# alibaba/unified-audio

Measured on AMD Instinct MI355X. Metric: audio-seconds/sec H-Codec encode+decode @16kHz b=32, higher is better.
Workload: dtype f32

## Files before the change

unified_audio_amd/csrc/conv_gemm.hip:

```cpp
#include <algorithm>
#include <cstdlib>
#include <type_traits>

#include "common.h"
#include "split_planes.h"

#ifndef QA_LOAD_AT
#define QA_LOAD_AT 0
#endif

#ifdef QA_TIMING
__device__ unsigned long long g_qa_timing[10];
extern "C" int qa_debug_timing(unsigned long long* out, int reset) {
    if (out && hipMemcpyFromSymbol(out, HIP_SYMBOL(g_qa_timing), sizeof(g_qa_timing)) != hipSuccess) return -1;
    if (reset) {
        unsigned long long z[10] = {0};
        if (hipMemcpyToSymbol(HIP_SYMBOL(g_qa_timing), z, sizeof(z)) != hipSuccess) return -1;
    }
    return 0;
}
#endif

namespace qa {

__host__ __device__ constexpr int conv_gemm_lds_bytes(int BM, int BN, int BK, bool split) {
    return (split ? 2 * (BM + BN) * 3 * BK * 2 : 2 * (BM + BN) * (BK + 4) * 4) + BM * 8 * 4;
}
__host__ __device__ constexpr int conv_gemm_min_wg(int BM, int BN, int BK, bool split) {
    const int regs = BM == 256 ? (BK == 16 ? 2 : 1) : (BM == 64 && (BK == 16 || BN == 64) ? 4 : (BK == 16 ? 3 : 2));
    const int lds = 160 * 1024 / conv_gemm_lds_bytes(BM, BN, BK, split);
    return regs < lds ? regs : (lds < 1 ? 1 : lds);
}

template <int N, int I = 0, class F>
__device__ __forceinline__ void static_for(F&& f) {
    if constexpr (I < N) {
        f(std::integral_constant<int, I>{});
        static_for<N, I + 1>(f);
    }
}

constexpr int TAP_WIN = 8;

__device__ __forceinline__ float snake_f(float x, float a) {
    const float s = sinf(a * x);
    return x + s * s / (a + 1e-9f);
}
__device__ __forceinline__ f32x4 snake4(f32x4 v, const float* alpha, int n) {
    const f32x4 a = *reinterpret_cast<const f32x4*>(alpha + n);
    const f32x4 r = {snake_f(v.x, a.x), snake_f(v.y, a.y), snake_f(v.z, a.z), snake_f(v.w, a.w)};
    return r;
}

__device__ __forceinline__ f32x4 epilogue4(f32x4 v, const ConvParams& p, long long m, int n, f32x4 bias, f32x4 gamma) {
    v += bias;
    if (p.gate) {
        const f32x4 g = *reinterpret_cast<const f32x4*>(p.gate + m * p.ldg + n);
        v.x *= silu_f(g.x); v.y *= silu_f(g.y); v.z *= silu_f(g.z); v.w *= silu_f(g.w);
    }
    if (p.act == ACT_SNAKE) {
        v = snake4(v, p.alpha, n);
    } else if (p.act != ACT_NONE) {
        v.x = apply_act(v.x, p.act); v.y = apply_act(v.y, p.act); v.z = apply_act(v.z, p.act); v.w = apply_act(v.w, p.act);
    }
    if (p.gamma) v *= gamma;
    if (p.res) v += *reinterpret_cast<const f32x4*>(p.res + m * p.ldr + n);
    if (p.post_act == ACT_SNAKE) {
        v = snake4(v, p.alpha, n);
    } else if (p.post_act != ACT_NONE) {
        v.x = apply_act(v.x, p.post_act); v.y = apply_act(v.y, p.post_act); v.z = apply_act(v.z, p.post_act);
        v.w = apply_act(v.w, p.post_act);
    }
    if (p.y2) *reinterpret_cast<f32x4*>(p.y2 + m * p.ldy2 + n) = snake4(v, p.alpha2, n);
    if (p.rope && n < p.rope_n) {
        const int t = p.rope_pos0 + (int)(m % p.rope_T), i = (n % p.rope_hd) >> 1;
        const f32x4 cs = *reinterpret_cast<const f32x4*>(p.rope + ((long long)t * (p.rope_hd >> 1) + i) * 2);
        const f32x4 r = {v.x * cs.x - v.y * cs.y, v.y * cs.x + v.x * cs.y, v.z * cs.z - v.w * cs.w, v.w * cs.z + v.z * cs.w};
        v = r;
    }
    return v;
}

template <int BM, int BN, int WM, int WN, bool PRO_ELU, int BK = 32, bool LINEAR = false, int NPL = 0, bool PRE = false>
__global__ __launch_bounds__(256, conv_gemm_min_wg(BM, BN, BK, NPL > 0)) void conv_gemm_kernel(const ConvParams p_in) {
    constexpr bool SPLIT = NPL > 0;
    constexpr int NP = SPLIT ? NPL : 3;
    static_assert(NPL >= 0 && NPL <= 3, "0 = fp32 chain, else the number of bf16 planes");
    static_assert(SPLIT || !PRE, "a pre-split weight image feeds the bf16-plane instances only");
    ConvParams p = p_in;
    constexpr int CK = SPLIT ? 32 : BK;
    constexpr bool ONE_BUF = SPLIT && BK == 16;
    constexpr int LDS = BK + 4;
    constexpr int RPP = 256 / (CK / 4);
    constexpr int WTM = BM / WM, WTN = BN / WN;
    constexpr int TM = WTM / 32, TN = WTN / 32;
    constexpr int A_IT = BM / RPP, B_IT = BN / RPP;
    static_assert(WM * WN == 4, "4 waves per workgroup");
    static_assert(TM >= 1 && TN >= 1, "wave tile must hold at least one 32x32 MFMA tile");

    constexpr int SMEM_FLOATS = SPLIT ? (ONE_BUF ? 1 : 2) * (BM + BN) * 3 * CK / 2 : 2 * (BM + BN) * LDS;
    __shared__ __attribute__((aligned(16))) float smem[SMEM_FLOATS];
    __shared__ int s_tap[BM * TAP_WIN];
    float* sA = smem;
    float* sB = smem + 2 * BM * LDS;
    constexpr int PLANE_A = BM * CK * 2, PLANE_B = BN * CK * 2;
    constexpr int BUF_BYTES = 3 * (PLANE_A + PLANE_B);
    char* const sbytes = reinterpret_cast<char*>(smem);
    auto swz = [](int row, int slot) { return slot ^ ((0 - (row >> 2)) & 3); };

    const int tid = threadIdx.x, lane = tid & 63, wave = tid >> 6;
    const int wm = wave / WN, wn = wave % WN;
    const int tiles_n = (p.N + BN - 1) / BN;
    int tile = blockIdx.x;
    if (p.xcd_swizzle) {
        const int nwg = gridDim.x, q = nwg >> 3, r = nwg & 7;
        const int xcd = tile & 7, local = tile >> 3;
        tile = (xcd < r ? xcd * (q + 1) : r * (q + 1) + (xcd - r) * q) + local;
    }
    int tm_i = tile / tiles_n, tn_i = tile % tiles_n;
    if (p.panel > 0 && tiles_n > p.panel) {
        const int tiles_m = (p.M + BM - 1) / BM;
        const int per_panel = tiles_m * p.panel;
        const int panel = tile / per_panel, r = tile - panel * per_panel;
        const int pw = min(p.panel, tiles_n - panel * p.panel);
        tm_i = r / pw;
        tn_i = panel * p.panel + (r - tm_i * pw);
    }
    const int m0 = tm_i * BM;
    const int n0 = tn_i * BN;

    const int ld_row = tid / (CK / 4);
    const int ld_c4 = (tid % (CK / 4)) * 4;
    const bool ld_hi = SPLIT && ld_c4 >= 16, bp_hi = (tid & 2) != 0;
    const bool k_tail = SPLIT && (p.K & 16) != 0;

    const bool reflect = p.pad_mode == PAD_REFLECT;
    const int ldx_i = (int)p.ldx;
    const int t_virtual = p.T_in * (p.in_rep > 1 ? p.in_rep : 1);
    const int dil = p.dilation > 1 ? p.dilation : 1;
    auto build_taps = [&](int jbase) {
        for (int e = tid; e < BM * TAP_WIN; e += 256) {
            const int row = e / TAP_WIN, j = jbase + (e % TAP_WIN);
            const int m = min(m0 + row, p.M - 1);
            const int t = m % p.T_out;
            int len = t_virtual, lp = p.Lp;
            if (p.lens) {
                len = min(p.lens[m / p.T_out] * p.len_mul, t_virtual);
                lp = len <= p.max_pad ? p.max_pad + 1 : len;
            }
            int r = t * p.stride - p.pad_left + j * dil;
            const int rr = r < 0 ? -r : (r >= lp ? 2 * (lp - 1) - r : r);
            r = reflect ? rr : r;
            const bool ok = r >= 0 && r < len && j < p.ksize;
            const unsigned ru = ok ? (unsigned)r : 0u;
            const unsigned src = __umulhi(ru, p.rep_magic) + ru * p.rep_one;
            s_tap[e] = ok ? (int)(src * (unsigned)ldx_i) : -1;
        }
    };
    if (!LINEAR) build_taps(0);
    int jbase = 0;

    const float* a_ptr[A_IT];
    int a_tab[A_IT];
#pragma unroll
    for (int i = 0; i < A_IT; ++i) {
        const int m = min(m0 + ld_row + RPP * i, p.M - 1);
        a_ptr[i] = LINEAR ? p.x + (long long)m * p.ldx + ld_c4 : p.x + (long long)(m / p.T_out) * p.T_in * p.ldx + ld_c4;
        a_tab[i] = (ld_row + RPP * i) * TAP_WIN;
    }
    const float* b_ptr[B_IT];
    if constexpr (!PRE) {
#pragma unroll
        for (int i = 0; i < B_IT; ++i) {
            const int n = min(n0 + ld_row + RPP * i, p.N - 1);
            b_ptr[i] = p.w + (long long)n * p.K + ld_c4;
        }
    }
    constexpr int BP_BLOCK = 16 * NP;
    constexpr int BP_UNITS = BN * CK / 128 * BP_BLOCK, BP_IT = PRE ? BP_UNITS / 256 : 1;
    static_assert(!PRE || (BN == 128 && BP_UNITS % 256 == 0), "the image path exists for the 128-column tiles: every thread moves BP_IT whole units");
    const char* bp_ptr[BP_IT];
    int bp_lds[BP_IT];
    if constexpr (PRE) {
#pragma unroll
        for (int i = 0; i < BP_IT; ++i) {
            const int u = tid + 256 * i, v = u % BP_BLOCK;
            const int pl = v >> 4, slot = v % (CK / 8);
            const int row = u / BP_BLOCK * (128 / CK) + (v & 15) / (CK / 8);
            const int n = min(n0 + row, p.N - 1);
            bp_ptr[i] = static_cast<const char*>(p.wp) + plane_byte_offset((long long)n * p.K + slot * 8, pl);
            bp_lds[i] = 3 * PLANE_A + pl * PLANE_B + row * CK * 2 + swz(row, slot) * 16;
        }
    }
    const int nk = (p.K + CK - 1) / CK;

    f32x16 acc[TM][TN];
#pragma unroll
    for (int i = 0; i < TM; ++i)
#pragma unroll
        for (int j = 0; j < TN; ++j)
#pragma unroll
            for (int r = 0; r < 16; ++r) acc[i][j][r] = 0.f;
    constexpr int TM16 = WTM / 16, TN16 = WTN / 16;
    f32x4 acc4[SPLIT ? TM16 : 1][SPLIT ? TN16 : 1];
    if constexpr (SPLIT) {
#pragma unroll
        for (int i = 0; i < TM16; ++i)
#pragma unroll
            for (int j = 0; j < TN16; ++j) acc4[i][j] = f32x4{0.f, 0.f, 0.f, 0.f};
    }

    f32x4 a_reg[A_IT], b_reg[B_IT];
    u32x4 bp_reg[BP_IT];
    float a_keep[A_IT];

#define QA_LOAD_GLOBAL(KC)                                                                                     \
    {                                                                                                          \
        const int k0_ = (KC) * CK;                                                                             \
        const bool tl_ = k_tail && (KC) == nk - 1;             \
        const int kt_ = k0_ - (tl_ && ld_hi ? 16 : 0);          \
        if (LINEAR) {                                                                                          \
            _Pragma("unroll") for (int i = 0; i < A_IT; ++i) a_reg[i] = *reinterpret_cast<const f32x4*>(a_ptr[i] + kt_); \
        } else {                                                                                               \
            const int j0_ = k0_ / p.C_in;                                                                      \
            const int c0_ = k0_ - j0_ * p.C_in;                                                                \
            int j1_ = j0_, c1_ = c0_;                                                                          \
            if (SPLIT && (p.C_in & 16)) {        \
                const int kh_ = tl_ ? k0_ : k0_ + 16;                                                          \
                j1_ = kh_ / p.C_in;                                                                            \
                c1_ = kh_ - j1_ * p.C_in - 16;                                                                 \
            }                                                                                                  \
            if (j1_ >= jbase + TAP_WIN) {                         \
                jbase = j0_;                                                                                   \
                build_taps(jbase);                                                                             \
                __syncthreads();                                                                               \
            }                                                                                                  \
            const int j_ = ld_hi ? j1_ : j0_, c_ = ld_hi ? c1_ : c0_;                                          \
            _Pragma("unroll") for (int i = 0; i < A_IT; ++i) {                                                 \
                const int off_ = s_tap[a_tab[i] + (j_ - jbase)];                                               \
                a_keep[i] = off_ >= 0 ? 1.f : 0.f;                                                             \
                a_reg[i] = *reinterpret_cast<const f32x4*>(a_ptr[i] + (max(off_, 0) + c_));                    \
            }                                                                                                  \
        }                                                                                                      \
        if constexpr (PRE) {                                                                                   \
            const long long bo_ = (long long)(KC) * (CK * 6) - (tl_ && bp_hi ? 2 * PLANE_GROUP_BYTES : 0);     \
            _Pragma("unroll") for (int i = 0; i < BP_IT; ++i)                                                  \
                bp_reg[i] = *reinterpret_cast<const u32x4*>(bp_ptr[i] + bo_);                                  \
        } else {                                                                                               \
            _Pragma("unroll") for (int i = 0; i < B_IT; ++i) b_reg[i] = *reinterpret_cast<const f32x4*>(b_ptr[i] + kt_); \
        }                                                                                                      \
    }
#define QA_STORE_LDS(BUF, KC)                                                                                  \
    { if constexpr (SPLIT) {                                                                                   \
        char* a_ = sbytes + (BUF) * BUF_BYTES;                                                                 \
        const int sl_ = ld_c4 >> 3, in_ = (ld_c4 & 7) * 2;                                                     \
        if (k_tail && (KC) == nk - 1) {        \
            const f32x4 z4_ = {0.f, 0.f, 0.f, 0.f};                                                            \
            const u32x4 zu_ = {0u, 0u, 0u, 0u};                                                                \
            _Pragma("unroll") for (int i = 0; i < A_IT; ++i) a_reg[i] = ld_hi ? z4_ : a_reg[i];                \
            if constexpr (PRE) {                                                                               \
                _Pragma("unroll") for (int i = 0; i < BP_IT; ++i) bp_reg[i] = bp_hi ? zu_ : bp_reg[i];         \
            } else {                                                                                           \
                _Pragma("unroll") for (int i = 0; i < B_IT; ++i) b_reg[i] = ld_hi ? z4_ : b_reg[i];            \
            }                                                                                                  \
        }                                                                                                      \
        _Pragma("unroll") for (int i = 0; i < A_IT; ++i) {                                                     \
            f32x4 v = LINEAR ? a_reg[i] : a_reg[i] * a_keep[i];                                                \
            if (PRO_ELU) {                                                                                     \
                v.x = elu_f(v.x); v.y = elu_f(v.y); v.z = elu_f(v.z); v.w = elu_f(v.w);                        \
            }                                                                                                  \
            u32x2 h_, m_, l_;                                                                                  \
            split4_planes<NP>(v, h_, m_, l_);                                                                  \
            const int r_ = ld_row + RPP * i, o_ = r_ * CK * 2 + swz(r_, sl_) * 16 + in_;                       \
            *reinterpret_cast<u32x2*>(a_ + o_) = h_;                                                           \
            if constexpr (NP >= 2) *reinterpret_cast<u32x2*>(a_ + PLANE_A + o_) = m_;                          \
            if constexpr (NP == 3) *reinterpret_cast<u32x2*>(a_ + 2 * PLANE_A + o_) = l_;                      \
        }                                                                                                      \
        if constexpr (PRE) {                                                                                   \
            _Pragma("unroll") for (int i = 0; i < BP_IT; ++i)                                                  \
                *reinterpret_cast<u32x4*>(a_ + bp_lds[i]) = bp_reg[i];                                         \
        } else {                                                                                               \
        char* b_ = a_ + 3 * PLANE_A;                                                                           \
        _Pragma("unroll") for (int i = 0; i < B_IT; ++i) {                                                     \
            u32x2 h_, m_, l_;                                                                                  \
            split4_planes<NP>(b_reg[i], h_, m_, l_);                                                           \
            const int r_ = ld_row + RPP * i, o_ = r_ * CK * 2 + swz(r_, sl_) * 16 + in_;                       \
            *reinterpret_cast<u32x2*>(b_ + o_) = h_;                                                           \
            if constexpr (NP >= 2) *reinterpret_cast<u32x2*>(b_ + PLANE_B + o_) = m_;                          \
            if constexpr (NP == 3) *reinterpret_cast<u32x2*>(b_ + 2 * PLANE_B + o_) = l_;                      \
        } }                                                                                                    \
    } else {                                                                                                   \
        float* a_ = sA + (BUF) * BM * LDS;                                                                     \
        float* b_ = sB + (BUF) * BN * LDS;                                                                     \
        _Pragma("unroll") for (int i = 0; i < A_IT; ++i) {                                                     \
            f32x4 v = LINEAR ? a_reg[i] : a_reg[i] * a_keep[i];                                                \
            if (PRO_ELU) {                                                                                     \
                v.x = elu_f(v.x); v.y = elu_f(v.y); v.z = elu_f(v.z); v.w = elu_f(v.w);                        \
            }                                                                                                  \
            *reinterpret_cast<f32x4*>(a_ + (ld_row + RPP * i) * LDS + ld_c4) = v;                              \
        }                                                                                                      \
        _Pragma("unroll") for (int i = 0; i < B_IT; ++i)                                                       \
            *reinterpret_cast<f32x4*>(b_ + (ld_row + RPP * i) * LDS + ld_c4) = b_reg[i];                       \
    } }

    __syncthreads();
    QA_LOAD_GLOBAL(0)
    QA_STORE_LDS(0, 0)
    __syncthreads();

    const int frag_row = lane & 31;
    const int frag_k = (lane >> 5) * 4;
#ifdef QA_TIMING
    const long long tbegin = __builtin_readcyclecounter();
    const unsigned long long rbegin = __builtin_amdgcn_s_memrealtime();
#endif
    constexpr int NKK = BK / 8;
    if constexpr (SPLIT) {
        constexpr int RB = BM == 256 ? 4 : 1;
        constexpr int STORE_J = TN16 > 1 ? 1 : 0;
        const int fr = lane & 15, sl = lane >> 4;
        int a_off[TM16], b_off[TN16];
#pragma unroll
        for (int i = 0; i < TM16; ++i) {
            const int r = wm * WTM + i * 16 + fr;
            a_off[i] = r * CK * 2 + swz(r, sl) * 16;
        }
#pragma unroll
        for (int j = 0; j < TN16; ++j) {
            const int r = wn * WTN + j * 16 + fr;
            b_off[j] = 3 * PLANE_A + r * CK * 2 + swz(r, sl) * 16;
        }
        for (int kc = 0; kc < nk; ++kc) {
            const int cur = ONE_BUF ? 0 : kc & 1;
            const int nxt = min(kc + 1, nk - 1);
            const char* base = sbytes + cur * BUF_BYTES;
            QA_LOAD_GLOBAL(nxt)
            static_for<RB>([&](auto rb_c) {
                constexpr int i0 = decltype(rb_c)::value * (TM16 / RB);
                bf16x8 af[NP][TM16 / RB];
#pragma unroll
                for (int pl = 0; pl < NP; ++pl)
#pragma unroll
                    for (int i = 0; i < TM16 / RB; ++i) af[pl][i] = *reinterpret_cast<const bf16x8*>(base + pl * PLANE_A + a_off[i0 + i]);
#pragma unroll
                for (int j = 0; j < TN16; ++j) {
                    bf16x8 bf[NP];
#pragma unroll
                    for (int pl = 0; pl < NP; ++pl) bf[pl] = *reinterpret_cast<const bf16x8*>(base + pl * PLANE_B + b_off[j]);
                    if (!ONE_BUF && i0 + TM16 / RB == TM16 && j == STORE_J) QA_STORE_LDS(cur ^ 1, nxt)
                    static_for<6>([&](auto q_c) {
                        constexpr int q = decltype(q_c)::value;
                        if constexpr (pair_kept(q, NP)) {
#pragma unroll
                            for (int i = 0; i < TM16 / RB; ++i)
                                acc4[i0 + i][j] = __builtin_amdgcn_mfma_f32_16x16x32_bf16(bf[PAIR_B[q]], af[PAIR_A[q]][i], acc4[i0 + i][j], 0, 0, 0);
                        }
                    });
                }
            });
            __builtin_amdgcn_sched_barrier(0);
            if constexpr (ONE_BUF) {
                if (kc + 1 < nk) {
                    __syncthreads();
                    QA_STORE_LDS(0, nxt)
                    __syncthreads();
                }
            } else {
                __syncthreads();
            }
        }
    } else
    for (int kc = 0; kc < nk; ++kc) {
        const int cur = kc & 1;
        const int nxt = min(kc + 1, nk - 1);
        const float* a = sA + cur * BM * LDS + (wm * WTM + frag_row) * LDS + frag_k;
        const float* b = sB + cur * BN * LDS + (wn * WTN + frag_row) * LDS + frag_k;
        f32x4 af[2][TM], bf[2][TN];
#pragma unroll
        for (int i = 0; i < TM; ++i) af[0][i] = *reinterpret_cast<const f32x4*>(a + i * 32 * LDS);
#pragma unroll
        for (int j = 0; j < TN; ++j) bf[0][j] = *reinterpret_cast<const f32x4*>(b + j * 32 * LDS);
#pragma unroll
        for (int kk = 0; kk < NKK; ++kk) {
            const int cb = kk & 1, nb = cb ^ 1;
            if (kk < NKK - 1) {
#pragma unroll
                for (int i = 0; i < TM; ++i) af[nb][i] = *reinterpret_cast<const f32x4*>(a + i * 32 * LDS + (kk + 1) * 8);
#pragma unroll
                for (int j = 0; j < TN; ++j) bf[nb][j] = *reinterpret_cast<const f32x4*>(b + j * 32 * LDS + (kk + 1) * 8);
            }
            if (kk == QA_LOAD_AT) QA_LOAD_GLOBAL(nxt)
            if (kk == NKK - 1) QA_STORE_LDS(cur ^ 1, nxt)
#pragma unroll
            for (int i = 0; i < TM; ++i)
#pragma unroll
                for (int j = 0; j < TN; ++j) {
                    acc[i][j] = __builtin_amdgcn_mfma_f32_32x32x2f32(bf[cb][j].x, af[cb][i].x, acc[i][j], 0, 0, 0);
                    acc[i][j] = __builtin_amdgcn_mfma_f32_32x32x2f32(bf[cb][j].y, af[cb][i].y, acc[i][j], 0, 0, 0);
                    acc[i][j] = __builtin_amdgcn_mfma_f32_32x32x2f32(bf[cb][j].z, af[cb][i].z, acc[i][j], 0, 0, 0);
                    acc[i][j] = __builtin_amdgcn_mfma_f32_32x32x2f32(bf[cb][j].w, af[cb][i].w, acc[i][j], 0, 0, 0);
                }
            __builtin_amdgcn_sched_barrier(0);
        }
        __syncthreads();
    }
#ifdef QA_TIMING
    const long long tloop = __builtin_readcyclecounter();
#endif
#undef QA_LOAD_GLOBAL
#undef QA_STORE_LDS

    constexpr int EP_LD = BN + 4;
    constexpr int EP_ROWS = WM * 32;
    constexpr int EP_C4 = BN / 4;
    static_assert(EP_ROWS * EP_LD <= 2 * (BM + BN) * LDS, "epilogue staging must fit in the operand buffers");
    static_assert(256 % EP_C4 == 0, "a thread keeps its column group across iterations");
    static_assert(EP_C4 % 8 == 0, "arg-min epilogue: the 8 lanes of a 32-column group are consecutive lanes of one wave");
    float* stage = smem;
    const int row_l = lane & 31, col_h = 4 * (lane >> 5);
    const int ep_c4 = tid % EP_C4, ep_r0 = tid / EP_C4;
    const int ep_n = n0 + 4 * ep_c4;
    const f32x4 zero4 = {0.f, 0.f, 0.f, 0.f}, one4 = {1.f, 1.f, 1.f, 1.f};
    f32x4 bias4 = zero4, gamma4 = one4;
    if (p.vec_epi && ep_n < p.N) {
        if (p.bias) bias4 = *reinterpret_cast<const f32x4*>(p.bias + ep_n);
        if (p.gamma) gamma4 = *reinterpret_cast<const f32x4*>(p.gamma + ep_n);
    }
    static_for<TM>([&](auto i_c) {
        constexpr int i = decltype(i_c)::value;
        __syncthreads();
        if constexpr (SPLIT) {
#pragma unroll
            for (int h = 0; h < 2; ++h)
#pragma unroll
                for (int j = 0; j < TN16; ++j)
                    *reinterpret_cast<f32x4*>(stage + (wm * 32 + h * 16 + (lane & 15)) * EP_LD + wn * WTN + j * 16 + 4 * (lane >> 4)) = acc4[2 * i + h][j];
        } else {
#pragma unroll
        for (int j = 0; j < TN; ++j)
#pragma unroll
            for (int g = 0; g < 4; ++g) {
                const f32x4 v = {acc[i][j][4 * g], acc[i][j][4 * g + 1], acc[i][j][4 * g + 2], acc[i][j][4 * g + 3]};
                *reinterpret_cast<f32x4*>(stage + (wm * 32 + row_l) * EP_LD + wn * WTN + j * 32 + 8 * g + col_h) = v;
            }
        }
        __syncthreads();
#pragma unroll 1
        for (int r = ep_r0; r < EP_ROWS; r += 256 / EP_C4) {
            const long long m = m0 + (r >> 5) * WTM + i * 32 + (r & 31);
            if (p.am_dist) {
                float best = INFINITY;
                int bi = 0x7fffffff;
                if (m < p.M && ep_n < p.N) {
                    const f32x4 sv = *reinterpret_cast<const f32x4*>(stage + r * EP_LD + 4 * ep_c4);
                    const f32x4 e4 = *reinterpret_cast<const f32x4*>(p.am_e2 + ep_n);
                    const float xx = p.am_x2[m];
#pragma unroll
                    for (int e = 0; e < 4; ++e) {
                        const float dist = (xx - 2.f * sv[e]) + e4[e];
                        if (dist < best) {
                            best = dist;
                            bi = ep_n + e;
                        }
                    }
                }
#pragma unroll
                for (int o = 1; o < 8; o <<= 1) {
                    const float d2 = __shfl_xor(best, o, 64);
                    const int i2 = __shfl_xor(bi, o, 64);
                    if (d2 < best || (d2 == best && i2 < bi)) {
                        best = d2;
                        bi = i2;
                    }
                }
                if ((ep_c4 & 7) == 0 && m < p.M && ep_n < p.N) {
                    p.am_dist[m * p.am_ld + (ep_n >> 5)] = best;
                    p.am_idx[m * p.am_ld + (ep_n >> 5)] = bi;
                }
                continue;
            }
            if (m >= p.M || ep_n >= p.N) continue;
            f32x4 v = *reinterpret_cast<const f32x4*>(stage + r * EP_LD + 4 * ep_c4);
            if (p.vec_epi) {
                v = epilogue4(v, p, m, ep_n, bias4, gamma4);
                *reinterpret_cast<f32x4*>(p.y + m * p.ldy + ep_n) = v;
            } else {
                for (int e = 0; e < 4 && ep_n + e < p.N; ++e) {
                    const int n = ep_n + e;
                    float u = v[e] + (p.bias ? p.bias[n] : 0.f);
                    if (p.gate) u = silu_f(p.gate[m * p.ldg + n]) * u;
                    u = apply_act(u, p.act);
                    if (p.gamma) u *= p.gamma[n];
                    if (p.res) u += p.res[m * p.ldr + n];
                    u = apply_act(u, p.post_act);
                    p.y[m * p.ldy + n] = u;
                }
            }
        }
    });
#ifdef QA_TIMING
    if (lane == 0) {
        const long long tend = __builtin_readcyclecounter();
        atomicAdd(&g_qa_timing[4], (unsigned long long)(tend - tloop));
        atomicAdd(&g_qa_timing[5], (unsigned long long)(tend - tbegin));
        atomicAdd(&g_qa_timing[6], 1ULL);
        atomicAdd(&g_qa_timing[7], (unsigned long long)nk);
        atomicAdd(&g_qa_timing[8], __builtin_amdgcn_s_memrealtime() - rbegin);
    }
#endif
}

static bool is_linear(const ConvParams& p) {
    return knob(K_GEMM_LINEAR) != 0 && p.ksize == 1 && p.stride == 1 && p.pad_left == 0 && p.in_rep <= 1 && p.T_in == p.T_out && p.dilation <= 1;
}

constexpr int prof_cfg(int bm, int bn) {
    return bm == 256 ? PROF_CFG_256x128 : bm == 64 ? (bn == 64 ? PROF_CFG_64x64 : PROF_CFG_64x128) : bn == 32 ? PROF_CFG_128x32 : bn == 64 ? PROF_CFG_128x64 : PROF_CFG_128x128;
}

static int gemm_planes(const ConvParams& p) {
    const long long math = knob(K_GEMM_MATH);
    return math == 0 || p.math_fp32 ? 0 : math == 2 ? 2 : math == 3 ? 1 : 3;
}

template <int BM, int BN, int WM, int WN, bool ELU, int BK, bool LIN>
static void launch_instance(const ConvParams& p, long long tiles, hipStream_t stream) {
    constexpr bool IMAGE = BN == 128;
    const bool image = IMAGE && p.wp;
    void (*kernel)(const ConvParams) = nullptr;
    switch (gemm_planes(p)) {
        case 0: kernel = conv_gemm_kernel<BM, BN, WM, WN, ELU, BK, LIN, 0, false>; break;
        case 1: kernel = image ? conv_gemm_kernel<BM, BN, WM, WN, ELU, BK, LIN, 1, IMAGE> : conv_gemm_kernel<BM, BN, WM, WN, ELU, BK, LIN, 1, false>; break;
        case 2: kernel = image ? conv_gemm_kernel<BM, BN, WM, WN, ELU, BK, LIN, 2, IMAGE> : conv_gemm_kernel<BM, BN, WM, WN, ELU, BK, LIN, 2, false>; break;
        default: kernel = image ? conv_gemm_kernel<BM, BN, WM, WN, ELU, BK, LIN, 3, IMAGE> : conv_gemm_kernel<BM, BN, WM, WN, ELU, BK, LIN, 3, false>; break;
    }
    hipLaunchKernelGGL(kernel, dim3((unsigned)tiles), dim3(256), 0, stream, p);
}

static thread_local int t_gemm_lanes = 1;
GemmLanes::GemmLanes(int n) : prev(t_gemm_lanes) { t_gemm_lanes = n > 1 ? n : 1; }
GemmLanes::~GemmLanes() { t_gemm_lanes = prev; }
static bool takes_bk16(int bm, int bn, long long tiles, int K, int C_in, bool elu) {
    return bm == 256 ||
           (bn >= 64 && !elu && ((K <= knob(K_GEMM_BK16) && tiles * t_gemm_lanes >= knob(K_GEMM_BK16_MIN_TILES)) || C_in % 32 != 0));
}

template <int BM, int BN, int WM, int WN>
static int launch_cfg(const ConvParams& p, hipStream_t stream) {
    QA_REQUIRE(p.prologue == ACT_NONE || p.prologue == ACT_ELU, "conv_gemm: prologue %d unsupported", p.prologue);
    const long long tiles = ceil_div(p.M, BM) * ceil_div(p.N, BN);
    const bool linear = is_linear(p), elu = p.prologue == ACT_ELU;
    const bool bk16 = takes_bk16(BM, BN, tiles, p.K, p.C_in, elu);
    const int bk = bk16 || gemm_planes(p) > 0 ? 16 : 32;
    const bool table = BM != 256 && (!linear || elu);
    QA_REQUIRE(p.K % bk == 0 && (!table || p.C_in % bk == 0),
               "conv_gemm: the %dx%d tile's K chunk needs K=%d / C_in=%d to be multiples of %d", BM, BN, p.K, p.C_in, bk);
    const bool prof = profile_enabled();
    if (prof) {
        const double n = p.algo_n ? p.algo_n : p.N, k = p.algo_k ? p.algo_k : p.K;
        const double out_elems = p.am_dist ? 2.0 * (double)p.M * p.am_ld + p.M + n
                                            : (double)p.M * n * (1.0 + (p.res ? 1.0 : 0.0) + (p.gate ? 1.0 : 0.0));
        const double elems = (double)p.B * p.T_in * p.C_in + n * k + out_elems;
        profile_record_begin(prof_cfg(BM, BN), 2.0 * (double)p.M * n * k, 4.0 * elems, stream, &p);
    }
    if constexpr (BM == 256) QA_REQUIRE(linear && !elu, "conv_gemm: the 256 x 128 tile exists for LINEAR layers only");
    constexpr int BK16 = BN >= 64 ? 16 : 32;
    if (bk16 && linear) launch_instance<BM, BN, WM, WN, false, BK16, true>(p, tiles, stream);
    else if constexpr (BM != 256) {
        if (bk16) launch_instance<BM, BN, WM, WN, false, BK16, false>(p, tiles, stream);
        else if (elu) launch_instance<BM, BN, WM, WN, true, 32, false>(p, tiles, stream);
        else if (linear) launch_instance<BM, BN, WM, WN, false, 32, true>(p, tiles, stream);
        else launch_instance<BM, BN, WM, WN, false, 32, false>(p, tiles, stream);
    }
    if (prof) profile_record_end(stream);
    QA_LAUNCH_CHECK();
    return QA_OK;
}

struct TileQuery {
    long long M, N, K;
    int C_in;
    bool lin, elu, split;
    bool image;
    int share;
};
static int workgroups_per_cu(int cfg, bool bk16, bool split) {
    switch (cfg) {
        case PROF_CFG_128x128: return bk16 ? 3 : split ? 1 : 2;
        case PROF_CFG_64x128: return bk16 ? 4 : 2;
        case PROF_CFG_128x64: return bk16 ? 4 : 2;
        case PROF_CFG_64x64: return bk16 ? 5 : split ? 3 : 4;
        case PROF_CFG_256x128: return 2;
        default: return split ? 2 : 3;
    }
}
static double tile_cost(const TileQuery& t, int cfg, int bm, int bn, double eff) {
    constexpr double kTile = 128.0 * 128.0, kRamp = 0.22, kLaunch = 0.27 * 512.0;
    const long long tiles = ceil_div(t.M, bm) * ceil_div(t.N, bn);
    const long long w = workgroups_per_cu(cfg, takes_bk16(bm, bn, tiles, (int)t.K, t.C_in, t.elu), t.split);
    const long long n = tiles * (t.share > 1 ? t.share : 1), cap = 256 * w;
    const long long rounds = ceil_div(n, cap), m = n - (rounds - 1) * cap;
    double last = 0.5 * ((double)ceil_div(m, 256) + (double)m / 256.0);
    if (last < 1.0) last = 1.0;
    return kTile * kLaunch + (double)t.K * ((double)bm * bn / eff * ((double)(w * (rounds - 1)) + last) + kRamp * kTile * (double)rounds);
}
static double tile_cost_r4(const TileQuery& t, int bm, int bn, double eff) {
    const long long tiles = ceil_div(t.M, bm) * ceil_div(t.N, bn);
    return (double)ceil_div(tiles, 256) * bm * bn / eff * (tiles <= 256 ? 1.25 : 1.0);
}
static int choose_tile(const TileQuery& t) {
    int cfg = (int)knob(K_GEMM_CFG);
    if (cfg < 0) {
        if (t.N <= 32) cfg = PROF_CFG_128x32;
        else if (t.N <= 64) cfg = PROF_CFG_128x64;
        else {
            struct Cand { int cfg, bm, bn; double eff6, eff32; };
            static const Cand cands[] = {{PROF_CFG_128x128, 128, 128, 1.0, 1.0}, {PROF_CFG_64x128, 64, 128, 0.85, 0.914},
                                         {PROF_CFG_128x64, 128, 64, 0.80, 0.913}, {PROF_CFG_64x64, 64, 64, 0.69, 0.871}};
            double best = 0.0;
            cfg = PROF_CFG_128x128;
            const long long eff256 = knob(K_GEMM_256);
            const bool r4 = t.split && !t.image;
            if (eff256 > 0 && t.lin && t.M >= 8000 && t.N >= 1024) {
                best = r4 ? tile_cost_r4(t, 256, 128, eff256 / 1000.0) : tile_cost(t, PROF_CFG_256x128, 256, 128, eff256 / 1000.0);
                cfg = PROF_CFG_256x128;
            }
            for (const Cand& c : cands) {
                const double cost = r4 ? tile_cost_r4(t, c.bm, c.bn, c.eff32) : tile_cost(t, c.cfg, c.bm, c.bn, t.split ? c.eff6 : c.eff32);
                if (best == 0.0 || cost < best * 0.995) {
                    best = cost;
                    cfg = c.cfg;
                }
            }
        }
    }
    if (cfg == PROF_CFG_128x32 && t.C_in % 32 != 0) return PROF_CFG_128x64;
    if ((cfg == PROF_CFG_256x128 && !t.lin) || cfg >= PROF_NCFG) return PROF_CFG_128x128;
    return cfg;
}
static int choose_tile(const ConvParams& p) {
    const bool elu = p.prologue == ACT_ELU;
    return choose_tile(TileQuery{p.M, p.N, p.K, p.C_in, is_linear(p) && !elu, elu, knob(K_GEMM_MATH) != 0 && !p.math_fp32, p.wp != nullptr, 1});
}

int launch_conv_gemm(const ConvParams& p, hipStream_t stream) {
    QA_REQUIRE(p.K % 16 == 0 && p.C_in % 16 == 0, "conv_gemm: K=%d / C_in=%d must be multiples of 16", p.K, p.C_in);
    QA_REQUIRE(p.C_in % 32 == 0 || gemm_planes(p) > 0 || (p.N > 32 && p.prologue != ACT_ELU),
               "conv_gemm: C_in=%d is not a multiple of 32 (the fp32 chain supports that only for N > 32 without the ELU prologue)", p.C_in);
    QA_REQUIRE((p.ldx % 4) == 0, "conv_gemm: ldx=%lld must be a multiple of 4 floats", p.ldx);
    QA_REQUIRE((long long)p.T_in * p.ldx < (1LL << 31), "conv_gemm: one batch item spans %lld floats (limit 2^31)",
               (long long)p.T_in * p.ldx);
    QA_REQUIRE(((uintptr_t)p.x % 16) == 0 && ((uintptr_t)p.w % 16) == 0, "conv_gemm: x / w must be 16-byte aligned");
    if (p.M <= 0 || p.N <= 0) return QA_OK;
    QA_REQUIRE(ceil_div(p.M, 64) * ceil_div(p.N, 32) < (1LL << 31), "conv_gemm: grid too large");
    auto al16 = [](const void* ptr) { return ((uintptr_t)ptr % 16) == 0; };
    const bool vec_epi = p.N % 4 == 0 && p.ldy % 4 == 0 && al16(p.y) && (!p.bias || al16(p.bias)) && (!p.gamma || al16(p.gamma)) &&
                         (!p.res || (p.ldr % 4 == 0 && al16(p.res))) && (!p.gate || (p.ldg % 4 == 0 && al16(p.gate)));
    QA_REQUIRE(p.in_rep <= 1 || p.pad_mode == PAD_ZERO, "conv_gemm: in_rep needs zero padding");
    const bool snake = p.act == ACT_SNAKE || p.post_act == ACT_SNAKE;
    QA_REQUIRE((!snake && !p.y2) || (vec_epi && (!snake || (p.alpha && al16(p.alpha))) &&
                                     (!p.y2 || (p.alpha2 && al16(p.alpha2) && al16(p.y2) && p.ldy2 % 4 == 0))),
               "conv_gemm: Snake activation / second output need the float4 epilogue and 16-byte aligned alpha vectors");
    QA_REQUIRE(p.dilation <= 1 || (p.pad_mode == PAD_ZERO && p.in_rep <= 1), "conv_gemm: dilation needs zero padding");
    QA_REQUIRE(!p.lens || (p.len_mul >= 1 && p.max_pad >= 0), "conv_gemm: per-clip lengths need len_mul >= 1");
    QA_REQUIRE(!p.am_dist || (vec_epi && p.am_idx && p.am_x2 && p.am_e2 && al16(p.am_e2) && p.am_ld >= (p.N + 31) / 32 && !p.y2),
               "conv_gemm: the arg-min epilogue needs N %% 4 == 0, x2 / e2 / dist / idx and am_ld >= ceil(N / 32)");
    QA_REQUIRE(!p.rope || (vec_epi && p.rope_hd % 4 == 0 && p.rope_n % 4 == 0 && p.rope_T > 0 && al16(p.rope)),
               "conv_gemm: fused RoPE needs the float4 epilogue (N, strides, pointers multiples of 4 / 16 B)");
    ConvParams q = p;
    q.xcd_swizzle = (int)knob(K_GEMM_XCD);
    q.panel = (int)knob(K_GEMM_PANEL);
    q.wp = knob(K_GEMM_PRESPLIT) != 0 ? weight_planes_find(p.w, (long long)p.N * p.K) : nullptr;
    q.vec_epi = vec_epi;
    q.rep_one = p.in_rep > 1 ? 0u : 1u;
    q.rep_magic = p.in_rep > 1 ? (unsigned)(((1ULL << 32) + p.in_rep - 1) / p.in_rep) : 0u;

    switch (choose_tile(q)) {
        case PROF_CFG_128x32: return launch_cfg<128, 32, 4, 1>(q, stream);
        case PROF_CFG_128x64: return launch_cfg<128, 64, 2, 2>(q, stream);
        case PROF_CFG_64x128: return launch_cfg<64, 128, 1, 4>(q, stream);
        case PROF_CFG_64x64: return launch_cfg<64, 64, 2, 2>(q, stream);
        case PROF_CFG_256x128: return launch_cfg<256, 128, 2, 2>(q, stream);
        default: return launch_cfg<128, 128, 2, 2>(q, stream);
    }
}

int conv_params_from_args(const qa_conv_args& a, ConvParams* out) {
    ConvParams p{};
    QA_REQUIRE(a.x && a.w && a.y, "conv1d_cl: x, w, y must be non-null");
    QA_REQUIRE(a.B > 0 && a.T_in > 0 && a.C_in > 0 && a.N > 0 && a.T_out >= 0, "conv1d_cl: bad shape");
    QA_REQUIRE(a.ksize >= 1 && a.stride >= 1 && a.pad_left >= 0 && a.pad_right >= 0, "conv1d_cl: bad geometry");
    QA_REQUIRE(a.B * a.T_out < (1LL << 31) && a.ksize * a.C_in < (1LL << 31), "conv1d_cl: shape too large");
    p.x = a.x; p.w = a.w; p.bias = a.bias; p.gamma = a.gamma; p.res = a.residual; p.gate = a.gate; p.y = a.y;
    p.ldx = a.ldx ? a.ldx : a.C_in;
    p.ldy = a.ldy ? a.ldy : a.N;
    p.ldr = a.ldr ? a.ldr : a.N;
    p.ldg = a.ldg ? a.ldg : a.N;
    p.B = (int)a.B; p.T_in = (int)a.T_in; p.C_in = (int)a.C_in; p.T_out = (int)a.T_out; p.N = (int)a.N;
    p.K = (int)(a.ksize * a.C_in);
    p.M = (int)(a.B * a.T_out);
    p.ksize = a.ksize; p.stride = a.stride; p.pad_left = a.pad_left; p.pad_mode = a.pad_mode;
    const int max_pad = a.pad_left > a.pad_right ? a.pad_left : a.pad_right;
    p.Lp = (p.T_in <= max_pad) ? max_pad + 1 : p.T_in;
    p.in_rep = a.in_rep > 1 ? a.in_rep : 1;
    QA_REQUIRE(a.T_out == 0 || (a.T_out - 1) * (int64_t)a.stride + a.ksize <= a.pad_left + a.T_in * (int64_t)p.in_rep + a.pad_right,
               "conv1d_cl: T_out=%lld windows do not fit pad_left=%d + T_in=%lld + pad_right=%d", (long long)a.T_out,
               a.pad_left, (long long)a.T_in, a.pad_right);
    p.prologue = a.prologue; p.act = a.act; p.post_act = a.post_act;
    *out = p;
    return QA_OK;
}

}

extern "C" int qa_debug_conv_gemm_tile(long long M, long long N, long long K, int ksize, int linear, int math_fp32, int share) {
    if (M <= 0 || N <= 0 || K <= 0 || ksize < 1 || K % ksize != 0 || M >= (1LL << 31) || N >= (1LL << 31) || K >= (1LL << 31)) {
        qa::set_error("qa_debug_conv_gemm_tile: bad argument");
        return -1;
    }
    const bool lin = linear != 0 && ksize == 1 && qa::knob(qa::K_GEMM_LINEAR) != 0;
    return qa::choose_tile(qa::TileQuery{M, N, K, (int)(K / ksize), lin, false, qa::knob(qa::K_GEMM_MATH) != 0 && !math_fp32, true, share});
}
```

Baseline: 3496.

## Fold clip offsets into tap table and pack padding mask into one register

The tap table now stores the full offset relative to the tile's first clip, so the conv A-loader keeps a single base pointer instead of A_IT per-row pointers and row-table indices. The per-row float keep factors become bits in one mask register, set with alignbit and applied as a select instead of a multiply. Separately, ELU-prologue 128x128 split layers may now take the BK16 instance. A host check keeps tile offsets within 32 bits, and a debug entry point is added. This is meant to cut VGPR pressure and address arithmetic in the hot load loop. The risk is that the new BK16 ELU instances behave differently or fail the offset limit on large inputs.

After: 3556, median of 6. 1.7% higher.

```diff
diff --git a/unified_audio_amd/csrc/conv_gemm.hip b/unified_audio_amd/csrc/conv_gemm.hip
--- a/unified_audio_amd/csrc/conv_gemm.hip
+++ b/unified_audio_amd/csrc/conv_gemm.hip
@@ -3,6 +3,7 @@
 #include <type_traits>
 
 #include "common.h"
+#include "conv_offsets.h"
 #include "split_planes.h"
 
 #ifndef QA_LOAD_AT
@@ -138,14 +139,16 @@
     const int ldx_i = (int)p.ldx;
     const int t_virtual = p.T_in * (p.in_rep > 1 ? p.in_rep : 1);
     const int dil = p.dilation > 1 ? p.dilation : 1;
+    const int clip0 = m0 / p.T_out;
+    const unsigned clip_stride = (unsigned)p.T_in * (unsigned)ldx_i;
     auto build_taps = [&](int jbase) {
         for (int e = tid; e < BM * TAP_WIN; e += 256) {
             const int row = e / TAP_WIN, j = jbase + (e % TAP_WIN);
             const int m = min(m0 + row, p.M - 1);
-            const int t = m % p.T_out;
+            const int clip = m / p.T_out, t = m - clip * p.T_out;
             int len = t_virtual, lp = p.Lp;
             if (p.lens) {
-                len = min(p.lens[m / p.T_out] * p.len_mul, t_virtual);
+                len = min(p.lens[clip] * p.len_mul, t_virtual);
                 lp = len <= p.max_pad ? p.max_pad + 1 : len;
             }
             int r = t * p.stride - p.pad_left + j * dil;
@@ -154,19 +157,19 @@
             const bool ok = r >= 0 && r < len && j < p.ksize;
             const unsigned ru = ok ? (unsigned)r : 0u;
             const unsigned src = __umulhi(ru, p.rep_magic) + ru * p.rep_one;
-            s_tap[e] = ok ? (int)(src * (unsigned)ldx_i) : -1;
+            s_tap[e] = ok ? (int)((unsigned)(clip - clip0) * clip_stride + src * (unsigned)ldx_i) : -1;
         }
     };
     if (!LINEAR) build_taps(0);
     int jbase = 0;
 
-    const float* a_ptr[A_IT];
-    int a_tab[A_IT];
-#pragma unroll
-    for (int i = 0; i < A_IT; ++i) {
-        const int m = min(m0 + ld_row + RPP * i, p.M - 1);
-        a_ptr[i] = LINEAR ? p.x + (long long)m * p.ldx + ld_c4 : p.x + (long long)(m / p.T_out) * p.T_in * p.ldx + ld_c4;
-        a_tab[i] = (ld_row + RPP * i) * TAP_WIN;
+    const float* a_ptr[LINEAR ? A_IT : 1];
+    const int a_tab0 = ld_row * TAP_WIN;
+    if constexpr (LINEAR) {
+#pragma unroll
+        for (int i = 0; i < A_IT; ++i) a_ptr[i] = p.x + (long long)min(m0 + ld_row + RPP * i, p.M - 1) * p.ldx + ld_c4;
+    } else {
+        a_ptr[0] = p.x + (long long)clip0 * p.T_in * p.ldx + ld_c4;
     }
     const float* b_ptr[B_IT];
     if constexpr (!PRE) {
@@ -212,7 +215,8 @@
 
     f32x4 a_reg[A_IT], b_reg[B_IT];
     u32x4 bp_reg[BP_IT];
-    float a_keep[A_IT];
+    static_assert(A_IT <= 32, "one mask register for the staged rows");
+    unsigned a_pad = 0u;
 
 #define QA_LOAD_GLOBAL(KC)                                                                                     \
     {                                                                                                          \
@@ -236,10 +240,12 @@
                 __syncthreads();                                                                               \
             }                                                                                                  \
             const int j_ = ld_hi ? j1_ : j0_, c_ = ld_hi ? c1_ : c0_;                                          \
+            const int* tab_ = s_tap + (a_tab0 + (j_ - jbase));                                                 \
+            const float* ac_ = a_ptr[0] + c_;                                                                  \
             _Pragma("unroll") for (int i = 0; i < A_IT; ++i) {                                                 \
-                const int off_ = s_tap[a_tab[i] + (j_ - jbase)];                                               \
-                a_keep[i] = off_ >= 0 ? 1.f : 0.f;                                                             \
-                a_reg[i] = *reinterpret_cast<const f32x4*>(a_ptr[i] + (max(off_, 0) + c_));                    \
+                const int off_ = tab_[i * RPP * TAP_WIN];                                                      \
+                a_pad = __builtin_amdgcn_alignbit(a_pad, (unsigned)off_, 31);         \
+                a_reg[i] = *reinterpret_cast<const f32x4*>(ac_ + (unsigned)max(off_, 0));                      \
             }                                                                                                  \
         }                                                                                                      \
         if constexpr (PRE) {                                                                                   \
@@ -265,7 +271,8 @@
             }                                                                                                  \
         }                                                                                                      \
         _Pragma("unroll") for (int i = 0; i < A_IT; ++i) {                                                     \
-            f32x4 v = LINEAR ? a_reg[i] : a_reg[i] * a_keep[i];                                                \
+            f32x4 v = a_reg[i];                                                                                \
+            if (!LINEAR && (a_pad >> (A_IT - 1 - i) & 1u)) v = f32x4{0.f, 0.f, 0.f, 0.f};                      \
             if (PRO_ELU) {                                                                                     \
                 v.x = elu_f(v.x); v.y = elu_f(v.y); v.z = elu_f(v.z); v.w = elu_f(v.w);                        \
             }                                                                                                  \
@@ -293,7 +300,8 @@
         float* a_ = sA + (BUF) * BM * LDS;                                                                     \
         float* b_ = sB + (BUF) * BN * LDS;                                                                     \
         _Pragma("unroll") for (int i = 0; i < A_IT; ++i) {                                                     \
-            f32x4 v = LINEAR ? a_reg[i] : a_reg[i] * a_keep[i];                                                \
+            f32x4 v = a_reg[i];                                                                                \
+            if (!LINEAR && (a_pad >> (A_IT - 1 - i) & 1u)) v = f32x4{0.f, 0.f, 0.f, 0.f};                      \
             if (PRO_ELU) {                                                                                     \
                 v.x = elu_f(v.x); v.y = elu_f(v.y); v.z = elu_f(v.z); v.w = elu_f(v.w);                        \
             }                                                                                                  \
@@ -524,25 +532,29 @@
 }
 
 template <int BM, int BN, int WM, int WN, bool ELU, int BK, bool LIN>
-static void launch_instance(const ConvParams& p, long long tiles, hipStream_t stream) {
+static int launch_instance(const ConvParams& p, long long tiles, hipStream_t stream) {
     constexpr bool IMAGE = BN == 128;
     const bool image = IMAGE && p.wp;
     void (*kernel)(const ConvParams) = nullptr;
     switch (gemm_planes(p)) {
-        case 0: kernel = conv_gemm_kernel<BM, BN, WM, WN, ELU, BK, LIN, 0, false>; break;
+        case 0:
+            if constexpr (!(ELU && BK == 16)) kernel = conv_gemm_kernel<BM, BN, WM, WN, ELU, BK, LIN, 0, false>;
+            break;
         case 1: kernel = image ? conv_gemm_kernel<BM, BN, WM, WN, ELU, BK, LIN, 1, IMAGE> : conv_gemm_kernel<BM, BN, WM, WN, ELU, BK, LIN, 1, false>; break;
         case 2: kernel = image ? conv_gemm_kernel<BM, BN, WM, WN, ELU, BK, LIN, 2, IMAGE> : conv_gemm_kernel<BM, BN, WM, WN, ELU, BK, LIN, 2, false>; break;
         default: kernel = image ? conv_gemm_kernel<BM, BN, WM, WN, ELU, BK, LIN, 3, IMAGE> : conv_gemm_kernel<BM, BN, WM, WN, ELU, BK, LIN, 3, false>; break;
     }
+    QA_REQUIRE(kernel != nullptr, "conv_gemm: no %dx%d kernel instance for this launch (ELU %d, BK %d)", BM, BN, (int)ELU, BK);
     hipLaunchKernelGGL(kernel, dim3((unsigned)tiles), dim3(256), 0, stream, p);
+    return QA_OK;
 }
 
 static thread_local int t_gemm_lanes = 1;
 GemmLanes::GemmLanes(int n) : prev(t_gemm_lanes) { t_gemm_lanes = n > 1 ? n : 1; }
 GemmLanes::~GemmLanes() { t_gemm_lanes = prev; }
-static bool takes_bk16(int bm, int bn, long long tiles, int K, int C_in, bool elu) {
-    return bm == 256 ||
-           (bn >= 64 && !elu && ((K <= knob(K_GEMM_BK16) && tiles * t_gemm_lanes >= knob(K_GEMM_BK16_MIN_TILES)) || C_in % 32 != 0));
+static bool takes_bk16(int bm, int bn, long long tiles, int K, int C_in, bool elu, bool split) {
+    return bm == 256 || (bn >= 64 && (!elu || (bm == 128 && bn == 128 && split)) &&
+                         ((K <= knob(K_GEMM_BK16) && tiles * t_gemm_lanes >= knob(K_GEMM_BK16_MIN_TILES)) || C_in % 32 != 0));
 }
 
 template <int BM, int BN, int WM, int WN>
@@ -550,11 +562,15 @@
     QA_REQUIRE(p.prologue == ACT_NONE || p.prologue == ACT_ELU, "conv_gemm: prologue %d unsupported", p.prologue);
     const long long tiles = ceil_div(p.M, BM) * ceil_div(p.N, BN);
     const bool linear = is_linear(p), elu = p.prologue == ACT_ELU;
-    const bool bk16 = takes_bk16(BM, BN, tiles, p.K, p.C_in, elu);
+    const bool bk16 = takes_bk16(BM, BN, tiles, p.K, p.C_in, elu, gemm_planes(p) > 0);
     const int bk = bk16 || gemm_planes(p) > 0 ? 16 : 32;
     const bool table = BM != 256 && (!linear || elu);
     QA_REQUIRE(p.K % bk == 0 && (!table || p.C_in % bk == 0),
                "conv_gemm: the %dx%d tile's K chunk needs K=%d / C_in=%d to be multiples of %d", BM, BN, p.K, p.C_in, bk);
+    int64_t span = 0;
+    QA_REQUIRE(!table || conv_tile_offsets_fit(BM, p.T_out, p.T_in, p.ldx, &span),
+               "conv_gemm: a %d-row tile spans %lld floats of x (%lld clips of T_in=%d x ldx=%lld; T_out=%d), limit 2^31", BM, (long long)span,
+               (long long)ceil_div(BM, p.T_out) + 1, p.T_in, (long long)p.ldx, p.T_out);
     const bool prof = profile_enabled();
     if (prof) {
         const double n = p.algo_n ? p.algo_n : p.N, k = p.algo_k ? p.algo_k : p.K;
@@ -565,14 +581,19 @@
     }
     if constexpr (BM == 256) QA_REQUIRE(linear && !elu, "conv_gemm: the 256 x 128 tile exists for LINEAR layers only");
     constexpr int BK16 = BN >= 64 ? 16 : 32;
-    if (bk16 && linear) launch_instance<BM, BN, WM, WN, false, BK16, true>(p, tiles, stream);
+    int rc = QA_OK;
+    if (bk16 && linear && !elu) rc = launch_instance<BM, BN, WM, WN, false, BK16, true>(p, tiles, stream);
     else if constexpr (BM != 256) {
-        if (bk16) launch_instance<BM, BN, WM, WN, false, BK16, false>(p, tiles, stream);
-        else if (elu) launch_instance<BM, BN, WM, WN, true, 32, false>(p, tiles, stream);
-        else if (linear) launch_instance<BM, BN, WM, WN, false, 32, true>(p, tiles, stream);
-        else launch_instance<BM, BN, WM, WN, false, 32, false>(p, tiles, stream);
+        if (bk16 && elu) {
+            QA_REQUIRE(BM == 128 && BN == 128, "conv_gemm: the one-buffer ELU instances exist for the 128 x 128 tile only");
+            if constexpr (BM == 128 && BN == 128) rc = launch_instance<BM, BN, WM, WN, true, 16, false>(p, tiles, stream);
+        } else if (bk16) rc = launch_instance<BM, BN, WM, WN, false, BK16, false>(p, tiles, stream);
+        else if (elu) rc = launch_instance<BM, BN, WM, WN, true, 32, false>(p, tiles, stream);
+        else if (linear) rc = launch_instance<BM, BN, WM, WN, false, 32, true>(p, tiles, stream);
+        else rc = launch_instance<BM, BN, WM, WN, false, 32, false>(p, tiles, stream);
     }
     if (prof) profile_record_end(stream);
+    if (rc != QA_OK) return rc;
     QA_LAUNCH_CHECK();
     return QA_OK;
 }
@@ -597,7 +618,7 @@
 static double tile_cost(const TileQuery& t, int cfg, int bm, int bn, double eff) {
     constexpr double kTile = 128.0 * 128.0, kRamp = 0.22, kLaunch = 0.27 * 512.0;
     const long long tiles = ceil_div(t.M, bm) * ceil_div(t.N, bn);
-    const long long w = workgroups_per_cu(cfg, takes_bk16(bm, bn, tiles, (int)t.K, t.C_in, t.elu), t.split);
+    const long long w = workgroups_per_cu(cfg, takes_bk16(bm, bn, tiles, (int)t.K, t.C_in, t.elu, t.split), t.split);
     const long long n = tiles * (t.share > 1 ? t.share : 1), cap = 256 * w;
     const long long rounds = ceil_div(n, cap), m = n - (rounds - 1) * cap;
     double last = 0.5 * ((double)ceil_div(m, 256) + (double)m / 256.0);
@@ -713,6 +734,22 @@
 
 }
 
+extern "C" int qa_debug_conv1d_cl_ex(const qa_conv_args* args, int dilation, const int* lens, int len_mul, void* stream) {
+    if (!args || dilation < 1) {
+        qa::set_error("qa_debug_conv1d_cl_ex: bad argument");
+        return QA_ERR_INVALID;
+    }
+    qa::ConvParams p;
+    QA_TRY(qa::conv_params_from_args(*args, &p));
+    p.dilation = dilation;
+    if (lens) {
+        p.lens = lens;
+        p.len_mul = len_mul;
+        p.max_pad = args->pad_left > args->pad_right ? args->pad_left : args->pad_right;
+    }
+    return qa::launch_conv_gemm(p, static_cast<hipStream_t>(stream));
+}
+
 extern "C" int qa_debug_conv_gemm_tile(long long M, long long N, long long K, int ksize, int linear, int math_fp32, int share) {
     if (M <= 0 || N <= 0 || K <= 0 || ksize < 1 || K % ksize != 0 || M >= (1LL << 31) || N >= (1LL << 31) || K >= (1LL << 31)) {
         qa::set_error("qa_debug_conv_gemm_tile: bad argument");
diff --git a/unified_audio_amd/csrc/conv_offsets.h b/unified_audio_amd/csrc/conv_offsets.h
--- /dev/null
+++ b/unified_audio_amd/csrc/conv_offsets.h
@@ -0,0 +1,23 @@
+#pragma once
+#include <cstdint>
+
+namespace qa {
+
+constexpr int64_t CONV_OFFSET_LIMIT = INT64_C(1) << 31;
+
+inline int64_t conv_tile_offset_span(int64_t bm, int64_t t_out, int64_t t_in, int64_t ldx) {
+    if (bm <= 0 || t_out <= 0 || t_in <= 0 || ldx <= 0) return 0;
+    const int64_t clips = bm / t_out + (bm % t_out != 0) + 1;
+    if (t_in > INT64_MAX / ldx) return INT64_MAX;
+    const int64_t clip = t_in * ldx;
+    if (clip > INT64_MAX / clips) return INT64_MAX;
+    return clips * clip;
+}
+
+inline bool conv_tile_offsets_fit(int64_t bm, int64_t t_out, int64_t t_in, int64_t ldx, int64_t* span) {
+    const int64_t s = conv_tile_offset_span(bm, t_out, t_in, ldx);
+    if (span) *span = s;
+    return s < CONV_OFFSET_LIMIT;
+}
+
+}
```
